# Jackie-Chou/MC-CNN-python

Measured on AMD Instinct MI355X. Metric: Mdisparities/s (HxWxD / s) end-to-end match.py timed region, images resident in HBM, higher is better.
Workload: dtype f32; 1 GPU; cfg2: 750x500 synthetic stereo pair, D=256, one pair per GPU; weights=converted reference checkpoint

## Files before the change

mc-cnn-python_amd/csrc/cost_volume.hip:

```cpp
#include "common.h"

namespace mccnn {

constexpr int CV_TW = 64;
constexpr int CV_DT = 64;
constexpr int CV_C = 64;
#ifndef CVM_WAVES_PER_SIMD
#define CVM_WAVES_PER_SIMD 6
#endif
constexpr int CV_LD = 68;

template <bool PIXEL_MAJOR>
__global__ __launch_bounds__(256) void cost_volume_exact_kernel(const float *__restrict__ fl,
                                                                const float *__restrict__ fr, int H, int W, int D,
                                                                float *__restrict__ lcv, float *__restrict__ rcv, int Dp)
{
    __shared__ __attribute__((aligned(16))) float sR[(CV_TW + CV_DT - 1) * CV_LD];
    __shared__ __attribute__((aligned(16))) float sL[CV_TW * CV_LD];
    const int w0 = blockIdx.x * CV_TW, h = blockIdx.y, d0 = blockIdx.z * CV_DT;
    if (w0 + CV_TW - 1 < d0) return;
    const int tid = threadIdx.x;
    const size_t rowbase = (size_t)h * W;
    for (int i = tid; i < CV_TW * 16; i += 256) {
        const int px = i >> 4, c4 = i & 15;
        float4 v = make_float4(0.f, 0.f, 0.f, 0.f);
        if (w0 + px < W) v = *reinterpret_cast<const float4 *>(fl + (rowbase + w0 + px) * CV_C + c4 * 4);
        *reinterpret_cast<float4 *>(&sL[px * CV_LD + c4 * 4]) = v;
    }
    const int xr0 = w0 - d0 - (CV_DT - 1);
    for (int i = tid; i < (CV_TW + CV_DT - 1) * 16; i += 256) {
        const int r = i >> 4, c4 = i & 15;
        const int x = xr0 + r;
        float4 v = make_float4(0.f, 0.f, 0.f, 0.f);
        if (x >= 0 && x < W) v = *reinterpret_cast<const float4 *>(fr + (rowbase + x) * CV_C + c4 * 4);
        *reinterpret_cast<float4 *>(&sR[r * CV_LD + c4 * 4]) = v;
    }
    __syncthreads();

    const int wl = tid & 63, dq = tid >> 6;
    const int w = w0 + wl;
    float a[CV_C];
#pragma unroll
    for (int c4 = 0; c4 < 16; ++c4) {
        const float4 v = *reinterpret_cast<const float4 *>(&sL[wl * CV_LD + c4 * 4]);
        a[c4 * 4 + 0] = v.x; a[c4 * 4 + 1] = v.y; a[c4 * 4 + 2] = v.z; a[c4 * 4 + 3] = v.w;
    }
    const size_t plane = (size_t)H * W;
    constexpr int TP = 65;
    float *const sT = sL;
    if (PIXEL_MAJOR) __syncthreads();
    for (int k = 0; k < 16; ++k) {
        const int d = d0 + dq * 16 + k;
        if (d >= D) break;
        const int r = wl + (CV_DT - 1) - (dq * 16 + k);
        if (w < W && w >= d) {
            const float *b = &sR[r * CV_LD];
            float acc[8];
#pragma unroll
            for (int i = 0; i < 8; ++i) {
                const float4 b0 = *reinterpret_cast<const float4 *>(b + i * 8);
                const float4 b1 = *reinterpret_cast<const float4 *>(b + i * 8 + 4);
                const float p0 = a[i * 8 + 0] * b0.x, p1 = a[i * 8 + 1] * b0.y, p2 = a[i * 8 + 2] * b0.z,
                            p3 = a[i * 8 + 3] * b0.w, p4 = a[i * 8 + 4] * b1.x, p5 = a[i * 8 + 5] * b1.y,
                            p6 = a[i * 8 + 6] * b1.z, p7 = a[i * 8 + 7] * b1.w;
                if (i == 0) {
                    acc[0] = p0; acc[1] = p1; acc[2] = p2; acc[3] = p3;
                    acc[4] = p4; acc[5] = p5; acc[6] = p6; acc[7] = p7;
                } else {
                    acc[0] += p0; acc[1] += p1; acc[2] += p2; acc[3] += p3;
                    acc[4] += p4; acc[5] += p5; acc[6] += p6; acc[7] += p7;
                }
            }
            float s = ((acc[0] + acc[1]) + (acc[2] + acc[3])) + ((acc[4] + acc[5]) + (acc[6] + acc[7]));
            s = 0.f + s;
            s = -1.f * s;
            if (PIXEL_MAJOR) {
                sT[wl * TP + dq * 16 + k] = s;
            } else {
                lcv[(size_t)d * plane + rowbase + w] = s;
                rcv[(size_t)d * plane + rowbase + (w - d)] = s;
            }
        }
    }
    if (PIXEL_MAJOR) {
        __syncthreads();
        const int nd = min(CV_DT, D - d0);
        const int dl = tid & 63;
        for (int px = tid >> 6; px < CV_TW; px += 4) {
            const int ww = w0 + px, d = d0 + dl;
            if (ww < W && dl < nd && ww >= d) lcv[(rowbase + ww) * (size_t)Dp + d] = sT[px * TP + dl];
        }
        for (int xi = tid >> 6; xi < CV_TW + CV_DT - 1; xi += 4) {
            const int x = xr0 + xi, d = d0 + dl, px = x + d - w0;
            if (x >= 0 && dl < nd && px >= 0 && px < CV_TW && w0 + px < W)
                rcv[(rowbase + x) * (size_t)Dp + d] = sT[px * TP + dl];
        }
    }
}

constexpr int CVP_TW = 63;
#ifndef CVP_ABL
#define CVP_ABL 0
#endif
__device__ __forceinline__ bool cvp_never(int D) { return D == 12345; }
__global__ __launch_bounds__(256, 3) void cost_volume_exact_pairs_kernel(const float *__restrict__ fl,
                                                                         const float *__restrict__ fr, int H, int W, int D,
                                                                         float *__restrict__ lcv, float *__restrict__ rcv,
                                                                         int Dp)
{
    constexpr int RING = 128;
    __shared__ __attribute__((aligned(16))) float sR[RING * CV_LD];
    __shared__ __attribute__((aligned(16))) float sL[CV_TW * CV_LD];
    const int w0 = (int)blockIdx.x * CVP_TW - 1, h = blockIdx.y;
    const int tid = threadIdx.x;
    const size_t rowbase = (size_t)h * W;
    for (int i = tid; i < CV_TW * 16; i += 256) {
        const int px = i >> 4, c4 = i & 15;
        float4 v = make_float4(0.f, 0.f, 0.f, 0.f);
        if (w0 + px >= 0 && w0 + px < W) v = *reinterpret_cast<const float4 *>(fl + (rowbase + w0 + px) * CV_C + c4 * 4);
        *reinterpret_cast<float4 *>(&sL[px * CV_LD + c4 * 4]) = v;
    }
    for (int i = tid; i < (CV_TW + CV_DT - 1) * 16; i += 256) {
        const int x = w0 - (CV_DT - 1) + (i >> 4), c4 = i & 15;
        float4 v = make_float4(0.f, 0.f, 0.f, 0.f);
        if (x >= 0 && x < W) v = *reinterpret_cast<const float4 *>(fr + (rowbase + x) * CV_C + c4 * 4);
        *reinterpret_cast<float4 *>(&sR[(x & (RING - 1)) * CV_LD + c4 * 4]) = v;
    }
    __syncthreads();

    const int wl = tid & 63, dq = tid >> 6;
    const int w = w0 + wl;
    float a[CV_C];
#pragma unroll
    for (int c4 = 0; c4 < 16; ++c4) {
        const float4 v = *reinterpret_cast<const float4 *>(&sL[wl * CV_LD + c4 * 4]);
        a[c4 * 4 + 0] = v.x; a[c4 * 4 + 1] = v.y; a[c4 * 4 + 2] = v.z; a[c4 * 4 + 3] = v.w;
    }
    constexpr int TP = CV_LD;
    float *const sT = sL;
    __syncthreads();
#pragma unroll 1
    for (int d0 = 0; d0 < D && w0 + CV_TW - 1 >= d0; d0 += CV_DT) {
        const bool more = d0 + CV_DT < D && w0 + CV_TW - 1 >= d0 + CV_DT;
        float4 nx[4];
#pragma unroll
        for (int q = 0; q < 4; ++q) {
            const int i = tid + q * 256, x = w0 - d0 - (2 * CV_DT - 1) + (i >> 4), c4 = i & 15;
            nx[q] = make_float4(0.f, 0.f, 0.f, 0.f);
            if (more && x >= 0 && x < W) nx[q] = *reinterpret_cast<const float4 *>(fr + (rowbase + x) * CV_C + c4 * 4);
        }
#pragma unroll 1
        for (int kk = 0; kk < (((CVP_ABL & 1) && !cvp_never(D)) ? 0 : 8); ++kk) {
            const int dloc = dq * 16 + 2 * kk;
            const int r = (w - d0 - dloc) & (RING - 1);
            const float *b = &sR[r * CV_LD];
            float acc[8], acn[8];
            float4 n0 = *reinterpret_cast<const float4 *>(b), n1 = *reinterpret_cast<const float4 *>(b + 4);
#pragma unroll
            for (int i = 0; i < 8; ++i) {
                const float bv[8] = {n0.x, n0.y, n0.z, n0.w, n1.x, n1.y, n1.z, n1.w};
                if (i < 7) {
                    n0 = *reinterpret_cast<const float4 *>(b + (i + 1) * 8);
                    n1 = *reinterpret_cast<const float4 *>(b + (i + 1) * 8 + 4);
                }
#pragma unroll
                for (int j = 0; j < 8; j += 4) {
                    if (i == 0) {
                        asm volatile("v_mul_f32 %0, %8, %12\n\tv_mul_f32 %1, %9, %13\n\tv_mul_f32 %2, %10, %14\n\tv_mul_f32 %3, %11, %15\n\t"
                                     "v_mul_f32_dpp %4, %12, %8 wave_shr:1 row_mask:0xf bank_mask:0xf bound_ctrl:1\n\t"
                                     "v_mul_f32_dpp %5, %13, %9 wave_shr:1 row_mask:0xf bank_mask:0xf bound_ctrl:1\n\t"
                                     "v_mul_f32_dpp %6, %14, %10 wave_shr:1 row_mask:0xf bank_mask:0xf bound_ctrl:1\n\t"
                                     "v_mul_f32_dpp %7, %15, %11 wave_shr:1 row_mask:0xf bank_mask:0xf bound_ctrl:1"
                                     : "=&v"(acc[j]), "=&v"(acc[j + 1]), "=&v"(acc[j + 2]), "=&v"(acc[j + 3]),
                                       "=&v"(acn[j]), "=&v"(acn[j + 1]), "=&v"(acn[j + 2]), "=&v"(acn[j + 3])
                                     : "v"(a[j]), "v"(a[j + 1]), "v"(a[j + 2]), "v"(a[j + 3]),
                                       "v"(bv[j]), "v"(bv[j + 1]), "v"(bv[j + 2]), "v"(bv[j + 3]));
                    } else {
                        float t0, t1, t2, t3;
                        asm volatile("v_mul_f32 %8, %12, %16\n\tv_mul_f32 %9, %13, %17\n\tv_mul_f32 %10, %14, %18\n\tv_mul_f32 %11, %15, %19\n\t"
                                     "v_add_f32 %0, %0, %8\n\tv_add_f32 %1, %1, %9\n\tv_add_f32 %2, %2, %10\n\tv_add_f32 %3, %3, %11\n\t"
                                     "v_mul_f32_dpp %8, %16, %12 wave_shr:1 row_mask:0xf bank_mask:0xf bound_ctrl:1\n\t"
                                     "v_mul_f32_dpp %9, %17, %13 wave_shr:1 row_mask:0xf bank_mask:0xf bound_ctrl:1\n\t"
                                     "v_mul_f32_dpp %10, %18, %14 wave_shr:1 row_mask:0xf bank_mask:0xf bound_ctrl:1\n\t"
                                     "v_mul_f32_dpp %11, %19, %15 wave_shr:1 row_mask:0xf bank_mask:0xf bound_ctrl:1\n\t"
                                     "v_add_f32 %4, %4, %8\n\tv_add_f32 %5, %5, %9\n\tv_add_f32 %6, %6, %10\n\tv_add_f32 %7, %7, %11"
                                     : "+v"(acc[j]), "+v"(acc[j + 1]), "+v"(acc[j + 2]), "+v"(acc[j + 3]),
                                       "+v"(acn[j]), "+v"(acn[j + 1]), "+v"(acn[j + 2]), "+v"(acn[j + 3]),
                                       "=&v"(t0), "=&v"(t1), "=&v"(t2), "=&v"(t3)
                                     : "v"(a[i * 8 + j]), "v"(a[i * 8 + j + 1]), "v"(a[i * 8 + j + 2]), "v"(a[i * 8 + j + 3]),
                                       "v"(bv[j]), "v"(bv[j + 1]), "v"(bv[j + 2]), "v"(bv[j + 3]));
                    }
                }
                __builtin_amdgcn_sched_barrier(0);
            }
            float s = ((acc[0] + acc[1]) + (acc[2] + acc[3])) + ((acc[4] + acc[5]) + (acc[6] + acc[7]));
            float sn = ((acn[0] + acn[1]) + (acn[2] + acn[3])) + ((acn[4] + acn[5]) + (acn[6] + acn[7]));
            s = 0.f + s;
            sn = 0.f + sn;
            s = -1.f * s;
            sn = -1.f * sn;
            const int d = d0 + dloc;
            if (wl >= 1 && w < W) {
                if (d < D && w >= d) sT[wl * TP + dloc] = s;
                if (d + 1 < D && w >= d + 1) sT[wl * TP + dloc + 1] = sn;
            }
        }
        __syncthreads();
#pragma unroll
        for (int q = 0; q < 4; ++q) {
            const int i = tid + q * 256, x = w0 - d0 - (2 * CV_DT - 1) + (i >> 4), c4 = i & 15;
            if (more) *reinterpret_cast<float4 *>(&sR[(x & (RING - 1)) * CV_LD + c4 * 4]) = nx[q];
        }
        const int nd = ((CVP_ABL & 2) && !cvp_never(D)) ? 0 : min(CV_DT, D - d0);
        const int xr0 = w0 - d0 - (CV_DT - 1);
        const int q4 = (tid & 15) * 4, sub = tid >> 4;
        for (int px = 1 + sub; px < CV_TW; px += 16) {
            const int ww = w0 + px, d = d0 + q4;
            if (ww >= W || q4 >= nd || ww < d) continue;
            const float4 v = *reinterpret_cast<const float4 *>(&sT[px * TP + q4]);
            float *dst = lcv + (rowbase + ww) * (size_t)Dp + d;
            if (q4 + 3 < nd && ww >= d + 3) {
                *reinterpret_cast<float4 *>(dst) = v;
            } else {
                const float e[4] = {v.x, v.y, v.z, v.w};
#pragma unroll
                for (int j = 0; j < 4; ++j)
                    if (q4 + j < nd && ww >= d + j) dst[j] = e[j];
            }
        }
        for (int xi = sub; xi < CV_TW + CV_DT - 1; xi += 16) {
            const int x = xr0 + xi, d = d0 + q4, px = x + d - w0;
            if (x < 0 || q4 >= nd || px + 3 < 1 || px >= CV_TW) continue;
            float *dst = rcv + (rowbase + x) * (size_t)Dp + d;
            if (q4 + 3 < nd && px >= 1 && px + 3 < CV_TW && w0 + px + 3 < W) {
                float4 v;
                v.x = sT[px * TP + q4];
                v.y = sT[(px + 1) * TP + q4 + 1];
                v.z = sT[(px + 2) * TP + q4 + 2];
                v.w = sT[(px + 3) * TP + q4 + 3];
                *reinterpret_cast<float4 *>(dst) = v;
            } else {
#pragma unroll
                for (int j = 0; j < 4; ++j)
                    if (q4 + j < nd && px + j >= 1 && px + j < CV_TW && w0 + px + j < W) dst[j] = sT[(px + j) * TP + q4 + j];
            }
        }
        __syncthreads();
    }
}

using f32x16 = __attribute__((ext_vector_type(16))) float;
typedef _Float16 cv_h8 __attribute__((ext_vector_type(8)));
typedef _Float16 cv_h4 __attribute__((ext_vector_type(4)));
constexpr int CVM_SP = 144;
constexpr int CVM_TP = 68;

__device__ __forceinline__ void cv_split4(const float4 v, cv_h4 &hi, cv_h4 &lo)
{
    const float x[4] = {__builtin_amdgcn_fmed3f(v.x * 1024.f, -65504.f, 65504.f),
                        __builtin_amdgcn_fmed3f(v.y * 1024.f, -65504.f, 65504.f),
                        __builtin_amdgcn_fmed3f(v.z * 1024.f, -65504.f, 65504.f),
                        __builtin_amdgcn_fmed3f(v.w * 1024.f, -65504.f, 65504.f)};
#pragma unroll
    for (int j = 0; j < 4; ++j) {
        const _Float16 h = (_Float16)x[j];
        hi[j] = h;
        lo[j] = (_Float16)(x[j] - (float)h);
    }
}

template <bool PIXEL_MAJOR>
__global__ __launch_bounds__(256, CVM_WAVES_PER_SIMD) void cost_volume_mfma_kernel(
    const float *__restrict__ fl, const float *__restrict__ fr, int H, int W, int D, float *__restrict__ lcv,
    float *__restrict__ rcv, int nwt, int nbands, int total, int Dp)
{
    constexpr int LDS_BYTES = (2 * 64 * CVM_SP > 64 * CVM_TP * 4) ? 2 * 64 * CVM_SP : 64 * CVM_TP * 4;
    __shared__ __attribute__((aligned(16))) char lds[LDS_BYTES];
    char *oL = lds, *oR = lds + 64 * CVM_SP;
    float *sT = reinterpret_cast<float *>(lds);
    int id;
    {
        const int b = blockIdx.x, qq = total >> 3, r = total & 7, xc = b & 7;
        id = (xc < r ? xc * (qq + 1) : r * (qq + 1) + (xc - r) * qq) + (b >> 3);
    }
    const int wt = id % nwt, band = (id / nwt) % nbands;
    const int h = id / (nwt * nbands);
    const int w0 = wt * 64;
    const int x0 = w0 - band * 64;
    if (x0 + 63 < 0) return;
    if (w0 - x0 - 63 >= D) return;
    const int tid = threadIdx.x;
    const size_t rowbase = (size_t)h * W;
    float4 vl[2][2], vr[2][2];
#pragma unroll
    for (int hf = 0; hf < 2; ++hf)
#pragma unroll
        for (int j = 0; j < 2; ++j) {
            const int p = j * 256 + tid, px = p >> 3, c4 = hf * 8 + (p & 7);
            vl[hf][j] = make_float4(0.f, 0.f, 0.f, 0.f);
            vr[hf][j] = make_float4(0.f, 0.f, 0.f, 0.f);
            if (w0 + px < W) vl[hf][j] = *reinterpret_cast<const float4 *>(fl + (rowbase + w0 + px) * CV_C + c4 * 4);
            const int x = x0 + px;
            if (x >= 0 && x < W) vr[hf][j] = *reinterpret_cast<const float4 *>(fr + (rowbase + x) * CV_C + c4 * 4);
        }
    const int wave = tid >> 6, lane = tid & 63;
    const int wr = (wave >> 1) * 32, wc = (wave & 1) * 32;
    f32x16 acc, acc2;
#pragma unroll
    for (int i = 0; i < 16; ++i) acc[i] = 0.f, acc2[i] = 0.f;
    const char *pa = oL + (wr + (lane & 31)) * CVM_SP + 16 * (lane >> 5);
    const char *pb = oR + (wc + (lane & 31)) * CVM_SP + 16 * (lane >> 5);
#pragma unroll
    for (int hf = 0; hf < 2; ++hf) {
        if (hf) __syncthreads();
#pragma unroll
        for (int j = 0; j < 2; ++j) {
            const int p = j * 256 + tid, px = p >> 3, c = p & 7;
            const int off = px * CVM_SP + (c >> 2) * 64 + (c & 3) * 8;
            cv_h4 hh, ll;
            cv_split4(vl[hf][j], hh, ll);
            *reinterpret_cast<cv_h4 *>(oL + off) = hh;
            *reinterpret_cast<cv_h4 *>(oL + off + 32) = ll;
            cv_split4(vr[hf][j], hh, ll);
            *reinterpret_cast<cv_h4 *>(oR + off) = hh;
            *reinterpret_cast<cv_h4 *>(oR + off + 32) = ll;
        }
        __syncthreads();
#pragma unroll
        for (int q = 0; q < 2; ++q) {
            const cv_h8 a_hi = *reinterpret_cast<const cv_h8 *>(pa + q * 64);
            const cv_h8 a_lo = *reinterpret_cast<const cv_h8 *>(pa + q * 64 + 32);
            const cv_h8 b_hi = *reinterpret_cast<const cv_h8 *>(pb + q * 64);
            const cv_h8 b_lo = *reinterpret_cast<const cv_h8 *>(pb + q * 64 + 32);
            acc2 = __builtin_amdgcn_mfma_f32_32x32x16_f16(a_lo, b_hi, acc2, 0, 0, 0);
            acc = __builtin_amdgcn_mfma_f32_32x32x16_f16(a_hi, b_hi, acc, 0, 0, 0);
            acc2 = __builtin_amdgcn_mfma_f32_32x32x16_f16(a_hi, b_lo, acc2, 0, 0, 0);
        }
    }
    __syncthreads();
    if (PIXEL_MAJOR) {
        constexpr int TP = 65;
#pragma unroll
        for (int rg = 0; rg < 16; ++rg) {
            const int row = wr + (rg & 3) + 8 * (rg >> 2) + 4 * (lane >> 5);
            const int col = wc + (lane & 31);
            sT[row * TP + col] = (acc[rg] + acc2[rg]) * (-1.f / 1048576.f);
        }
        __syncthreads();
        const int dbase = w0 - x0;
        for (int r = wave; r < 64; r += 4) {
            const int w = w0 + r, d = dbase + r - lane;
            if (w < W && d >= 0 && d < D && w >= d) lcv[(rowbase + w) * (size_t)Dp + d] = sT[r * TP + lane];
        }
        for (int c = wave; c < 64; c += 4) {
            const int x = x0 + c, d = dbase + lane - c;
            if (x >= 0 && w0 + lane < W && d >= 0 && d < D) rcv[(rowbase + x) * (size_t)Dp + d] = sT[lane * TP + c];
        }
        return;
    }
#pragma unroll
    for (int rg = 0; rg < 16; ++rg) {
        const int row = wr + (rg & 3) + 8 * (rg >> 2) + 4 * (lane >> 5);
        const int col = wc + (lane & 31);
        sT[((row - col) & 63) * CVM_TP + row] = (acc[rg] + acc2[rg]) * (-1.f / 1048576.f);
    }
    __syncthreads();
    const size_t plane = (size_t)H * W;
    const int dbase = w0 - x0;
    typedef float f4u __attribute__((ext_vector_type(4), aligned(4)));
    const int q = lane & 15, sub = lane >> 4;
    for (int rgp = wave; rgp < 16; rgp += 4) {
        const int row = rgp * 4 + sub;
        const int wl = 4 * q;
        const float4 t = *reinterpret_cast<const float4 *>(&sT[row * CVM_TP + wl]);
        const float v[4] = {t.x, t.y, t.z, t.w};
        const int w = w0 + wl;
        if (wl >= row || wl + 3 < row) {
            const int dd = wl >= row ? row : row - 64;
            const int d = dbase + dd;
            if (d < 0 || d >= D || w >= W) continue;
            float *pl = lcv + (size_t)d * plane + rowbase + w;
            float *pr = rcv + (size_t)d * plane + rowbase + (w - d);
            if (w + 3 < W) {
                f4u o;
                o[0] = v[0]; o[1] = v[1]; o[2] = v[2]; o[3] = v[3];
                *reinterpret_cast<f4u *>(pl) = o;
                *reinterpret_cast<f4u *>(pr) = o;
            } else {
#pragma unroll
                for (int j = 0; j < 4; ++j)
                    if (w + j < W) {
                        pl[j] = v[j];
                        pr[j] = v[j];
                    }
            }
        }
    }
    {
        const int row = tid >> 2, j = tid & 3;
        const int c = (row & ~3) + j;
        const int d = dbase + (c >= row ? row : row - 64);
        const int w = w0 + c;
        if ((row & 3) != 0 && d >= 0 && d < D && w < W) {
            const float v = sT[row * CVM_TP + c];
            lcv[(size_t)d * plane + rowbase + w] = v;
            rcv[(size_t)d * plane + rowbase + (w - d)] = v;
        }
    }
}

__global__ __launch_bounds__(64) void cost_volume_fill_kernel(float *__restrict__ lcv, float *__restrict__ rcv, int D,
                                                              int H, int W)
{
    __shared__ float tile[64 * 65];
    const int lane = threadIdx.x;
    const int d = D - 1 - blockIdx.y;
    const int h0 = blockIdx.x * 64;
    const int h = min(h0 + lane, H - 1);
    const int nrows = min(64, H - h0);
    if (blockIdx.z == 0) {
        float *L = lcv + ((size_t)d * H + h) * W;
        float x1 = L[d], x2 = L[d + 1], x3 = L[d + 2];
        for (int wtop = d - 1; wtop >= 0; wtop -= 64) {
            const int cnt = min(64, wtop + 1);
            for (int j = 0; j < cnt; ++j) {
                float s = 0.f - x1;
                s = s - x2;
                s = s - x3;
                const float v = -(s / 3.f);
                tile[lane * 65 + j] = v;
                x3 = x2; x2 = x1; x1 = v;
            }
            __syncthreads();
            if (lane < cnt)
                for (int r = 0; r < nrows; ++r)
                    lcv[((size_t)d * H + h0 + r) * W + (wtop - lane)] = tile[r * 65 + lane];
            __syncthreads();
        }
    } else {
        float *Rr = rcv + ((size_t)d * H + h) * W;
        float x1 = Rr[W - d - 3], x2 = Rr[W - d - 2], x3 = Rr[W - d - 1];
        for (int wbot = W - d; wbot < W; wbot += 64) {
            const int cnt = min(64, W - wbot);
            for (int j = 0; j < cnt; ++j) {
                float s = 0.f - x1;
                s = s - x2;
                s = s - x3;
                const float v = -(s / 3.f);
                tile[lane * 65 + j] = v;
                x1 = x2; x2 = x3; x3 = v;
            }
            __syncthreads();
            if (lane < cnt)
                for (int r = 0; r < nrows; ++r)
                    rcv[((size_t)d * H + h0 + r) * W + (wbot + lane)] = tile[r * 65 + lane];
            __syncthreads();
        }
    }
}

typedef uint32_t cv_u32x4 __attribute__((ext_vector_type(4)));
template <int NG>
__global__ __launch_bounds__(64) void cost_volume_fill_hwd_kernel(float *__restrict__ lcv, float *__restrict__ rcv, int D,
                                                                  int Dp, int H, int W)
{
    constexpr int PF = 8;
    constexpr int kDrop = 0x7ffffff0;
    const int lane = threadIdx.x, h = blockIdx.x;
    const bool left = blockIdx.y == 0;
    float *row = (left ? lcv : rcv) + (size_t)h * W * Dp;
    const __amdgpu_buffer_rsrc_t rs = __builtin_amdgcn_make_buffer_rsrc(row, 0, (int)((size_t)W * Dp * 4), 0x00020000);
    const unsigned pix = (unsigned)Dp * 4u;
    const int c_first = left ? D + 1 : max(W - D - 2, 0), nsteps = left ? D + 2 : W - c_first;
    auto col = [&](int t) { return left ? c_first - t : c_first + t; };
    int dbase[NG], voff[NG];
    float x1[NG][4], x2[NG][4], x3[NG][4];
#pragma unroll
    for (int g = 0; g < NG; ++g) {
        dbase[g] = g * 256 + lane * 4;
        voff[g] = dbase[g] < Dp ? dbase[g] * 4 : kDrop;
#pragma unroll
        for (int i = 0; i < 4; ++i) x1[g][i] = x2[g][i] = x3[g][i] = 0.f;
    }
    cv_u32x4 buf[PF][NG];
    auto issue = [&](int slot, int t) {
        const unsigned so = (unsigned)col(min(t, nsteps - 1)) * pix;
#pragma unroll
        for (int g = 0; g < NG; ++g) buf[slot][g] = __builtin_amdgcn_raw_buffer_load_b128(rs, voff[g], so, 0);
    };
#pragma unroll
    for (int k = 0; k < PF; ++k) issue(k, k);
    for (int t0 = 0; t0 < nsteps; t0 += PF) {
#pragma unroll
        for (int k = 0; k < PF; ++k) {
            const int t = t0 + k;
            if (t >= nsteps) continue;
            const int c = col(t);
#pragma unroll
            for (int g = 0; g < NG; ++g) {
                const cv_u32x4 u = buf[k][g];
                const float v[4] = {__uint_as_float(u.x), __uint_as_float(u.y), __uint_as_float(u.z), __uint_as_float(u.w)};
                cv_u32x4 o;
                bool any = false;
#pragma unroll
                for (int i = 0; i < 4; ++i) {
                    const int d = dbase[g] + i;
                    const bool stored = left ? c >= d : c < W - d;
                    float s = 0.f - x1[g][i];
                    s = s - x2[g][i];
                    s = s - x3[g][i];
                    const float val = stored ? v[i] : -(s / 3.f);
                    any |= !stored && d < D;
                    if (left) { x3[g][i] = x2[g][i]; x2[g][i] = x1[g][i]; x1[g][i] = val; }
                    else      { x1[g][i] = x2[g][i]; x2[g][i] = x3[g][i]; x3[g][i] = val; }
                    o[i] = __float_as_uint(val);
                }
                buffer_store_b128<0>(o, rs, any ? voff[g] : kDrop, (unsigned)c * pix);
            }
            issue(k, t + PF);
        }
    }
}


__global__ __launch_bounds__(64) void cost_volume_fill_hwd_lanes_kernel(float *__restrict__ lcv, float *__restrict__ rcv,
                                                                        int D, int Dp, int H, int W)
{
    constexpr int PF = 16;
    constexpr int kDrop = 0x7ffffff0;
    const int lane = threadIdx.x, h = blockIdx.x;
    const bool left = blockIdx.y == 0;
    const int d = (int)blockIdx.z * 64 + lane;
    const int dmax = min((int)blockIdx.z * 64 + 63, D - 1);
    if ((int)blockIdx.z * 64 >= D) return;
    float *row = (left ? lcv : rcv) + (size_t)h * W * Dp;
    const __amdgpu_buffer_rsrc_t rs = __builtin_amdgcn_make_buffer_rsrc(row, 0, (int)((size_t)W * Dp * 4), 0x00020000);
    const unsigned pix = (unsigned)Dp * 4u;
    const int c_first = left ? dmax + 2 : max(W - dmax - 3, 0), nsteps = left ? c_first + 1 : W - c_first;
    auto col = [&](int t) { return left ? c_first - t : c_first + t; };
    const int voff = d < Dp ? d * 4 : kDrop;
    const int sto = d < D ? voff : kDrop;
    float x1 = 0.f, x2 = 0.f, x3 = 0.f;
    float buf[PF];
    const int dmin = (int)blockIdx.z * 64;
    const int nA = min(nsteps, left ? c_first - dmin + 1 : (W - dmin) - c_first);
    auto issue = [&](int slot, int t) {
        const int c = col(min(t, nA - 1));
        buf[slot] = __uint_as_float(__builtin_amdgcn_raw_buffer_load_b32(rs, voff, (unsigned)c * pix, 0));
    };
    auto third = [](float s) {
        const float zh = 0.3333333432674407958984375f;
        const float q = s * zh;
        const float r = __builtin_fmaf(-3.0f, q, s);
        const float q2 = __builtin_fmaf(r, zh, q);
        return (__builtin_fabsf(s) < __builtin_inff() && s != 0.f) ? q2 : s;
    };
    auto step = [&](int c, bool stored, float have) {
        float s = 0.f - x1;
        s = s - x2;
        s = s - x3;
        const float val = stored ? have : -third(s);
        if (left) { x3 = x2; x2 = x1; x1 = val; }
        else      { x1 = x2; x2 = x3; x3 = val; }
        __builtin_amdgcn_raw_buffer_store_b32(__float_as_uint(val), rs, stored ? kDrop : sto, (unsigned)c * pix, 0);
    };
    if (nA > 0) {
#pragma unroll
        for (int k = 0; k < PF; ++k) issue(k, k);
        for (int t0 = 0; t0 < nA; t0 += PF) {
#pragma unroll
            for (int k = 0; k < PF; ++k) {
                const int t = t0 + k;
                if (t < nA) {
                    const int c = col(t);
                    step(c, left ? c >= d : c < W - d, buf[k]);
                }
                issue(k, t + PF);
            }
        }
    }
    for (int t = max(nA, 0); t < nsteps; ++t) step(col(t), false, 0.f);
}

}

extern "C" int mccnn_cost_volume(const float *fl, const float *fr, int H, int W, int C, int D, float *lcv, float *rcv,
                                 int mode, mccnn_stream_t stream)
{
    using namespace mccnn;
    MCCNN_REQUIRE(fl && fr && lcv && rcv, MCCNN_E_INVALID, "mccnn_cost_volume: null pointer");
    MCCNN_REQUIRE(H > 0 && W > 0 && D > 0, MCCNN_E_INVALID, "mccnn_cost_volume: non-positive size");
    MCCNN_REQUIRE(C == CV_C, MCCNN_E_UNSUPPORTED, "mccnn_cost_volume: C=%d, kernels are built for 64 channels", C);
    MCCNN_REQUIRE(D <= W - 2, MCCNN_E_UNSUPPORTED,
                  "mccnn_cost_volume: D=%d needs W >= D+2 (the reference's border recurrence pf:106 is degenerate "
                  "beyond that), W=%d", D, W);
    hipStream_t s = (hipStream_t)stream;
    const dim3 block(256);
    if (mode == MCCNN_CV_EXACT) {
        const dim3 grid(cdiv(W, CV_TW), H, cdiv(D, CV_DT));
        hipLaunchKernelGGL(cost_volume_exact_kernel<false>, grid, block, 0, s, fl, fr, H, W, D, lcv, rcv, 0);
    } else if (mode == MCCNN_CV_MFMA) {
        const int nwt = cdiv(W, 64), nbands = cdiv(D + 63, 64) + 1;
        const long total = (long)nwt * nbands * H;
        MCCNN_REQUIRE(total <= 0x7fffffffL, MCCNN_E_UNSUPPORTED, "mccnn_cost_volume: %ld tiles exceed the grid", total);
        hipLaunchKernelGGL(cost_volume_mfma_kernel<false>, dim3((unsigned)total), block, 0, s, fl, fr, H, W, D, lcv, rcv, nwt,
                           nbands, (int)total, 0);
    } else {
        MCCNN_REQUIRE(false, MCCNN_E_INVALID, "mccnn_cost_volume: unknown mode %d", mode);
    }
    int rc = check_launch("mccnn_cost_volume");
    if (rc) return rc;
    if (D > 1)
        hipLaunchKernelGGL(cost_volume_fill_kernel, dim3(cdiv(H, 64), D - 1, 2), dim3(64), 0, s, lcv, rcv, D, H, W);
    return check_launch("mccnn_cost_volume(fill)");
}

extern "C" int mccnn_cost_volume_hwd(const float *fl, const float *fr, int H, int W, int C, int D, float *lcv_hwd,
                                     float *rcv_hwd, int mode, mccnn_stream_t stream)
{
    using namespace mccnn;
    MCCNN_REQUIRE(fl && fr && lcv_hwd && rcv_hwd, MCCNN_E_INVALID, "mccnn_cost_volume_hwd: null pointer");
    MCCNN_REQUIRE(H > 0 && W > 0 && D > 0, MCCNN_E_INVALID, "mccnn_cost_volume_hwd: non-positive size");
    MCCNN_REQUIRE(C == CV_C, MCCNN_E_UNSUPPORTED, "mccnn_cost_volume_hwd: C=%d, kernels are built for 64 channels", C);
    MCCNN_REQUIRE(D <= W - 2, MCCNN_E_UNSUPPORTED,
                  "mccnn_cost_volume_hwd: D=%d needs W >= D+2 (the reference's border recurrence pf:106 is degenerate "
                  "beyond that), W=%d", D, W);
    MCCNN_REQUIRE(mode == MCCNN_CV_EXACT || mode == MCCNN_CV_MFMA, MCCNN_E_INVALID, "mccnn_cost_volume_hwd: unknown mode %d",
                  mode);
    MCCNN_REQUIRE(D <= 512, MCCNN_E_UNSUPPORTED, "mccnn_cost_volume_hwd: D=%d > 512", D);
    const int Dp = mccnn_hwd_pitch(D);
    MCCNN_REQUIRE((size_t)W * Dp * 4 < ((size_t)1 << 31), MCCNN_E_UNSUPPORTED,
                  "mccnn_cost_volume_hwd: a %d x %d row exceeds a buffer descriptor's reach", W, D);
    hipStream_t s = (hipStream_t)stream;
    if (mode == MCCNN_CV_MFMA) {
        const int nwt = cdiv(W, 64), nbands = cdiv(D + 63, 64) + 1;
        const long total = (long)nwt * nbands * H;
        MCCNN_REQUIRE(total <= 0x7fffffffL, MCCNN_E_UNSUPPORTED, "mccnn_cost_volume_hwd: %ld tiles exceed the grid", total);
        hipLaunchKernelGGL(cost_volume_mfma_kernel<true>, dim3((unsigned)total), dim3(256), 0, s, fl, fr, H, W, D, lcv_hwd,
                           rcv_hwd, nwt, nbands, (int)total, Dp);
    } else {
#ifdef CV_HWD_TILE_KERNEL
        const dim3 grid(cdiv(W, CV_TW), H, cdiv(D, CV_DT));
        hipLaunchKernelGGL(cost_volume_exact_kernel<true>, grid, dim3(256), 0, s, fl, fr, H, W, D, lcv_hwd, rcv_hwd, Dp);
#else
        const dim3 grid(cdiv(W, CVP_TW), H, 1);
        hipLaunchKernelGGL(cost_volume_exact_pairs_kernel, grid, dim3(256), 0, s, fl, fr, H, W, D, lcv_hwd, rcv_hwd, Dp);
#endif
    }
    int rc = check_launch("mccnn_cost_volume_hwd");
    if (rc) return rc;
    if (D > 1) {
#ifdef CV_FILL_FOUR_PER_LANE
        if (Dp <= 256)
            hipLaunchKernelGGL(cost_volume_fill_hwd_kernel<1>, dim3(H, 2), dim3(64), 0, s, lcv_hwd, rcv_hwd, D, Dp, H, W);
        else
            hipLaunchKernelGGL(cost_volume_fill_hwd_kernel<2>, dim3(H, 2), dim3(64), 0, s, lcv_hwd, rcv_hwd, D, Dp, H, W);
#else
        hipLaunchKernelGGL(cost_volume_fill_hwd_lanes_kernel, dim3(H, 2, cdiv(D, 64)), dim3(64), 0, s, lcv_hwd, rcv_hwd, D, Dp,
                           H, W);
#endif
    }
    return check_launch("mccnn_cost_volume_hwd(fill)");
}
```

Measured before the change: 11340 Mdisparities/s.

## Add double-buffered rows cost-volume kernel overlapping score stores with compute

Adds a new exact cost-volume kernel that works in 32-disparity bands with two score tiles in shared memory. It interleaves the global stores of the previous band's scores (left and right volumes) with the dot-product computation of the current band, which cuts the per-band barrier-separated store phase. The shared pair-score inner loop is factored into a helper, and the old pairs kernel stays reachable behind a compile flag. The trade-off is more loop iterations, smaller tiles, and extra bounds logic in the store path.

```diff
diff --git a/mc-cnn-python_amd/csrc/cost_volume.hip b/mc-cnn-python_amd/csrc/cost_volume.hip
--- a/mc-cnn-python_amd/csrc/cost_volume.hip
+++ b/mc-cnn-python_amd/csrc/cost_volume.hip
@@ -103,6 +103,56 @@
 #define CVP_ABL 0
 #endif
 __device__ __forceinline__ bool cvp_never(int D) { return D == 12345; }
+
+__device__ __forceinline__ void cvp_pair_scores(const float *b, const float (&a)[CV_C], float &s, float &sn)
+{
+    float acc[8], acn[8];
+    float4 n0 = *reinterpret_cast<const float4 *>(b), n1 = *reinterpret_cast<const float4 *>(b + 4);
+#pragma unroll
+    for (int i = 0; i < 8; ++i) {
+        const float bv[8] = {n0.x, n0.y, n0.z, n0.w, n1.x, n1.y, n1.z, n1.w};
+        if (i < 7) {
+            n0 = *reinterpret_cast<const float4 *>(b + (i + 1) * 8);
+            n1 = *reinterpret_cast<const float4 *>(b + (i + 1) * 8 + 4);
+        }
+#pragma unroll
+        for (int j = 0; j < 8; j += 4) {
+            if (i == 0) {
+                asm volatile("v_mul_f32 %0, %8, %12\n\tv_mul_f32 %1, %9, %13\n\tv_mul_f32 %2, %10, %14\n\tv_mul_f32 %3, %11, %15\n\t"
+                             "v_mul_f32_dpp %4, %12, %8 wave_shr:1 row_mask:0xf bank_mask:0xf bound_ctrl:1\n\t"
+                             "v_mul_f32_dpp %5, %13, %9 wave_shr:1 row_mask:0xf bank_mask:0xf bound_ctrl:1\n\t"
+                             "v_mul_f32_dpp %6, %14, %10 wave_shr:1 row_mask:0xf bank_mask:0xf bound_ctrl:1\n\t"
+                             "v_mul_f32_dpp %7, %15, %11 wave_shr:1 row_mask:0xf bank_mask:0xf bound_ctrl:1"
+                             : "=&v"(acc[j]), "=&v"(acc[j + 1]), "=&v"(acc[j + 2]), "=&v"(acc[j + 3]),
+                               "=&v"(acn[j]), "=&v"(acn[j + 1]), "=&v"(acn[j + 2]), "=&v"(acn[j + 3])
+                             : "v"(a[j]), "v"(a[j + 1]), "v"(a[j + 2]), "v"(a[j + 3]),
+                               "v"(bv[j]), "v"(bv[j + 1]), "v"(bv[j + 2]), "v"(bv[j + 3]));
+            } else {
+                float t0, t1, t2, t3;
+                asm volatile("v_mul_f32 %8, %12, %16\n\tv_mul_f32 %9, %13, %17\n\tv_mul_f32 %10, %14, %18\n\tv_mul_f32 %11, %15, %19\n\t"
+                             "v_add_f32 %0, %0, %8\n\tv_add_f32 %1, %1, %9\n\tv_add_f32 %2, %2, %10\n\tv_add_f32 %3, %3, %11\n\t"
+                             "v_mul_f32_dpp %8, %16, %12 wave_shr:1 row_mask:0xf bank_mask:0xf bound_ctrl:1\n\t"
+                             "v_mul_f32_dpp %9, %17, %13 wave_shr:1 row_mask:0xf bank_mask:0xf bound_ctrl:1\n\t"
+                             "v_mul_f32_dpp %10, %18, %14 wave_shr:1 row_mask:0xf bank_mask:0xf bound_ctrl:1\n\t"
+                             "v_mul_f32_dpp %11, %19, %15 wave_shr:1 row_mask:0xf bank_mask:0xf bound_ctrl:1\n\t"
+                             "v_add_f32 %4, %4, %8\n\tv_add_f32 %5, %5, %9\n\tv_add_f32 %6, %6, %10\n\tv_add_f32 %7, %7, %11"
+                             : "+v"(acc[j]), "+v"(acc[j + 1]), "+v"(acc[j + 2]), "+v"(acc[j + 3]),
+                               "+v"(acn[j]), "+v"(acn[j + 1]), "+v"(acn[j + 2]), "+v"(acn[j + 3]),
+                               "=&v"(t0), "=&v"(t1), "=&v"(t2), "=&v"(t3)
+                             : "v"(a[i * 8 + j]), "v"(a[i * 8 + j + 1]), "v"(a[i * 8 + j + 2]), "v"(a[i * 8 + j + 3]),
+                               "v"(bv[j]), "v"(bv[j + 1]), "v"(bv[j + 2]), "v"(bv[j + 3]));
+            }
+        }
+        __builtin_amdgcn_sched_barrier(0);
+    }
+    s = ((acc[0] + acc[1]) + (acc[2] + acc[3])) + ((acc[4] + acc[5]) + (acc[6] + acc[7]));
+    sn = ((acn[0] + acn[1]) + (acn[2] + acn[3])) + ((acn[4] + acn[5]) + (acn[6] + acn[7]));
+    s = 0.f + s;
+    sn = 0.f + sn;
+    s = -1.f * s;
+    sn = -1.f * sn;
+}
+
 __global__ __launch_bounds__(256, 3) void cost_volume_exact_pairs_kernel(const float *__restrict__ fl,
                                                                          const float *__restrict__ fr, int H, int W, int D,
                                                                          float *__restrict__ lcv, float *__restrict__ rcv,
@@ -153,52 +203,8 @@
         for (int kk = 0; kk < (((CVP_ABL & 1) && !cvp_never(D)) ? 0 : 8); ++kk) {
             const int dloc = dq * 16 + 2 * kk;
             const int r = (w - d0 - dloc) & (RING - 1);
-            const float *b = &sR[r * CV_LD];
-            float acc[8], acn[8];
-            float4 n0 = *reinterpret_cast<const float4 *>(b), n1 = *reinterpret_cast<const float4 *>(b + 4);
-#pragma unroll
-            for (int i = 0; i < 8; ++i) {
-                const float bv[8] = {n0.x, n0.y, n0.z, n0.w, n1.x, n1.y, n1.z, n1.w};
-                if (i < 7) {
-                    n0 = *reinterpret_cast<const float4 *>(b + (i + 1) * 8);
-                    n1 = *reinterpret_cast<const float4 *>(b + (i + 1) * 8 + 4);
-                }
-#pragma unroll
-                for (int j = 0; j < 8; j += 4) {
-                    if (i == 0) {
-                        asm volatile("v_mul_f32 %0, %8, %12\n\tv_mul_f32 %1, %9, %13\n\tv_mul_f32 %2, %10, %14\n\tv_mul_f32 %3, %11, %15\n\t"
-                                     "v_mul_f32_dpp %4, %12, %8 wave_shr:1 row_mask:0xf bank_mask:0xf bound_ctrl:1\n\t"
-                                     "v_mul_f32_dpp %5, %13, %9 wave_shr:1 row_mask:0xf bank_mask:0xf bound_ctrl:1\n\t"
-                                     "v_mul_f32_dpp %6, %14, %10 wave_shr:1 row_mask:0xf bank_mask:0xf bound_ctrl:1\n\t"
-                                     "v_mul_f32_dpp %7, %15, %11 wave_shr:1 row_mask:0xf bank_mask:0xf bound_ctrl:1"
-                                     : "=&v"(acc[j]), "=&v"(acc[j + 1]), "=&v"(acc[j + 2]), "=&v"(acc[j + 3]),
-                                       "=&v"(acn[j]), "=&v"(acn[j + 1]), "=&v"(acn[j + 2]), "=&v"(acn[j + 3])
-                                     : "v"(a[j]), "v"(a[j + 1]), "v"(a[j + 2]), "v"(a[j + 3]),
-                                       "v"(bv[j]), "v"(bv[j + 1]), "v"(bv[j + 2]), "v"(bv[j + 3]));
-                    } else {
-                        float t0, t1, t2, t3;
-                        asm volatile("v_mul_f32 %8, %12, %16\n\tv_mul_f32 %9, %13, %17\n\tv_mul_f32 %10, %14, %18\n\tv_mul_f32 %11, %15, %19\n\t"
-                                     "v_add_f32 %0, %0, %8\n\tv_add_f32 %1, %1, %9\n\tv_add_f32 %2, %2, %10\n\tv_add_f32 %3, %3, %11\n\t"
-                                     "v_mul_f32_dpp %8, %16, %12 wave_shr:1 row_mask:0xf bank_mask:0xf bound_ctrl:1\n\t"
-                                     "v_mul_f32_dpp %9, %17, %13 wave_shr:1 row_mask:0xf bank_mask:0xf bound_ctrl:1\n\t"
-                                     "v_mul_f32_dpp %10, %18, %14 wave_shr:1 row_mask:0xf bank_mask:0xf bound_ctrl:1\n\t"
-                                     "v_mul_f32_dpp %11, %19, %15 wave_shr:1 row_mask:0xf bank_mask:0xf bound_ctrl:1\n\t"
-                                     "v_add_f32 %4, %4, %8\n\tv_add_f32 %5, %5, %9\n\tv_add_f32 %6, %6, %10\n\tv_add_f32 %7, %7, %11"
-                                     : "+v"(acc[j]), "+v"(acc[j + 1]), "+v"(acc[j + 2]), "+v"(acc[j + 3]),
-                                       "+v"(acn[j]), "+v"(acn[j + 1]), "+v"(acn[j + 2]), "+v"(acn[j + 3]),
-                                       "=&v"(t0), "=&v"(t1), "=&v"(t2), "=&v"(t3)
-                                     : "v"(a[i * 8 + j]), "v"(a[i * 8 + j + 1]), "v"(a[i * 8 + j + 2]), "v"(a[i * 8 + j + 3]),
-                                       "v"(bv[j]), "v"(bv[j + 1]), "v"(bv[j + 2]), "v"(bv[j + 3]));
-                    }
-                }
-                __builtin_amdgcn_sched_barrier(0);
-            }
-            float s = ((acc[0] + acc[1]) + (acc[2] + acc[3])) + ((acc[4] + acc[5]) + (acc[6] + acc[7]));
-            float sn = ((acn[0] + acn[1]) + (acn[2] + acn[3])) + ((acn[4] + acn[5]) + (acn[6] + acn[7]));
-            s = 0.f + s;
-            sn = 0.f + sn;
-            s = -1.f * s;
-            sn = -1.f * sn;
+            float s, sn;
+            cvp_pair_scores(&sR[r * CV_LD], a, s, sn);
             const int d = d0 + dloc;
             if (wl >= 1 && w < W) {
                 if (d < D && w >= d) sT[wl * TP + dloc] = s;
@@ -247,6 +253,126 @@
         }
         __syncthreads();
     }
+}
+
+constexpr int CVR_DT = 32;
+constexpr int CVR_TP = 34;
+constexpr int CVR_SLOTS = 5;
+
+__device__ __forceinline__ void cvr_store_slot(int s, const float *__restrict__ sP, int tid, int w0, int pd0, int D, int W,
+                                               int Dp, size_t rowbase, float *__restrict__ lcv, float *__restrict__ rcv)
+{
+    const int nd = min(CVR_DT, D - pd0);
+    if (s < 2) {
+        const int slot = tid + s * 256, px = slot >> 3, q4 = (slot & 7) * 4;
+        const int ww = w0 + px, d = pd0 + q4;
+        if (px < 1 || ww >= W || q4 >= nd || ww < d) return;
+        const float2 lo = *reinterpret_cast<const float2 *>(&sP[px * CVR_TP + q4]);
+        const float2 hi = *reinterpret_cast<const float2 *>(&sP[px * CVR_TP + q4 + 2]);
+        float *dst = lcv + (rowbase + ww) * (size_t)Dp + d;
+        if (q4 + 3 < nd && ww >= d + 3) {
+            *reinterpret_cast<float4 *>(dst) = make_float4(lo.x, lo.y, hi.x, hi.y);
+        } else {
+            const float e[4] = {lo.x, lo.y, hi.x, hi.y};
+#pragma unroll
+            for (int j = 0; j < 4; ++j)
+                if (q4 + j < nd && ww >= d + j) dst[j] = e[j];
+        }
+    } else {
+        const int slot = tid + (s - 2) * 256, xi = slot >> 3, q4 = (slot & 7) * 4;
+        const int x = w0 - pd0 - (CVR_DT - 1) + xi, d = pd0 + q4, px = xi - (CVR_DT - 1) + q4;
+        if (xi >= CV_TW + CVR_DT - 1 || x < 0 || q4 >= nd || px + 3 < 1 || px >= CV_TW) return;
+        float *dst = rcv + (rowbase + x) * (size_t)Dp + d;
+        if (q4 + 3 < nd && px >= 1 && px + 3 < CV_TW && w0 + px + 3 < W) {
+            float4 v;
+            v.x = sP[px * CVR_TP + q4];
+            v.y = sP[(px + 1) * CVR_TP + q4 + 1];
+            v.z = sP[(px + 2) * CVR_TP + q4 + 2];
+            v.w = sP[(px + 3) * CVR_TP + q4 + 3];
+            *reinterpret_cast<float4 *>(dst) = v;
+        } else {
+#pragma unroll
+            for (int j = 0; j < 4; ++j)
+                if (q4 + j < nd && px + j >= 1 && px + j < CV_TW && w0 + px + j < W) dst[j] = sP[(px + j) * CVR_TP + q4 + j];
+        }
+    }
+}
+
+__global__ __launch_bounds__(256, 3) void cost_volume_exact_rows_kernel(const float *__restrict__ fl,
+                                                                        const float *__restrict__ fr, int H, int W, int D,
+                                                                        float *__restrict__ lcv, float *__restrict__ rcv,
+                                                                        int Dp)
+{
+    constexpr int RING = 128;
+    constexpr int TILE = CV_TW * CVR_TP;
+    static_assert(2 * TILE >= CV_TW * CV_LD, "the left features live where the score tiles go");
+    static_assert((CV_TW + 2 * CVR_DT - 1) <= RING, "a tile's columns and the next tile's new ones share the ring");
+    __shared__ __attribute__((aligned(16))) float sR[RING * CV_LD];
+    __shared__ __attribute__((aligned(16))) float sT2[2 * TILE];
+    float *const sL = sT2;
+    const int w0 = (int)blockIdx.x * CVP_TW - 1, h = blockIdx.y;
+    const int tid = threadIdx.x;
+    const size_t rowbase = (size_t)h * W;
+    for (int i = tid; i < CV_TW * 16; i += 256) {
+        const int px = i >> 4, c4 = i & 15;
+        float4 v = make_float4(0.f, 0.f, 0.f, 0.f);
+        if (w0 + px >= 0 && w0 + px < W) v = *reinterpret_cast<const float4 *>(fl + (rowbase + w0 + px) * CV_C + c4 * 4);
+        *reinterpret_cast<float4 *>(&sL[px * CV_LD + c4 * 4]) = v;
+    }
+    for (int i = tid; i < (CV_TW + CVR_DT - 1) * 16; i += 256) {
+        const int x = w0 - (CVR_DT - 1) + (i >> 4), c4 = i & 15;
+        float4 v = make_float4(0.f, 0.f, 0.f, 0.f);
+        if (x >= 0 && x < W) v = *reinterpret_cast<const float4 *>(fr + (rowbase + x) * CV_C + c4 * 4);
+        *reinterpret_cast<float4 *>(&sR[(x & (RING - 1)) * CV_LD + c4 * 4]) = v;
+    }
+    __syncthreads();
+
+    const int wl = tid & 63, dq = tid >> 6;
+    const int w = w0 + wl;
+    float a[CV_C];
+#pragma unroll
+    for (int c4 = 0; c4 < 16; ++c4) {
+        const float4 v = *reinterpret_cast<const float4 *>(&sL[wl * CV_LD + c4 * 4]);
+        a[c4 * 4 + 0] = v.x; a[c4 * 4 + 1] = v.y; a[c4 * 4 + 2] = v.z; a[c4 * 4 + 3] = v.w;
+    }
+    __syncthreads();
+    int pd0 = -1;
+    int buf = 0;
+#pragma unroll 1
+    for (int d0 = 0; d0 < D && w0 + CV_TW - 1 >= d0; d0 += CVR_DT) {
+        const bool more = d0 + CVR_DT < D && w0 + CV_TW - 1 >= d0 + CVR_DT;
+        float4 nx[2];
+#pragma unroll
+        for (int q = 0; q < 2; ++q) {
+            const int i = tid + q * 256, x = w0 - d0 - (2 * CVR_DT - 1) + (i >> 4), c4 = i & 15;
+            nx[q] = make_float4(0.f, 0.f, 0.f, 0.f);
+            if (more && x >= 0 && x < W) nx[q] = *reinterpret_cast<const float4 *>(fr + (rowbase + x) * CV_C + c4 * 4);
+        }
+        float *const sT = sT2 + buf * TILE;
+        const float *const sP = sT2 + (buf ^ 1) * TILE;
+#pragma unroll
+        for (int kk = 0; kk < 4; ++kk) {
+            if (pd0 >= 0)
+                for (int s = kk + (kk >= 2); s < kk + 1 + (kk + 1 >= 2); ++s)
+                    cvr_store_slot(s, sP, tid, w0, pd0, D, W, Dp, rowbase, lcv, rcv);
+            const int dloc = dq * 8 + 2 * kk;
+            if (d0 + dloc < D) {
+                float s, sn;
+                cvp_pair_scores(&sR[((w - d0 - dloc) & (RING - 1)) * CV_LD], a, s, sn);
+                *reinterpret_cast<float2 *>(&sT[wl * CVR_TP + dloc]) = make_float2(s, sn);
+            }
+        }
+#pragma unroll
+        for (int q = 0; q < 2; ++q) {
+            const int i = tid + q * 256, x = w0 - d0 - (2 * CVR_DT - 1) + (i >> 4), c4 = i & 15;
+            if (more) *reinterpret_cast<float4 *>(&sR[(x & (RING - 1)) * CV_LD + c4 * 4]) = nx[q];
+        }
+        __syncthreads();
+        pd0 = d0;
+        buf ^= 1;
+    }
+    if (pd0 >= 0)
+        for (int s = 0; s < CVR_SLOTS; ++s) cvr_store_slot(s, sT2 + (buf ^ 1) * TILE, tid, w0, pd0, D, W, Dp, rowbase, lcv, rcv);
 }
 
 using f32x16 = __attribute__((ext_vector_type(16))) float;
@@ -642,9 +768,12 @@
 #ifdef CV_HWD_TILE_KERNEL
         const dim3 grid(cdiv(W, CV_TW), H, cdiv(D, CV_DT));
         hipLaunchKernelGGL(cost_volume_exact_kernel<true>, grid, dim3(256), 0, s, fl, fr, H, W, D, lcv_hwd, rcv_hwd, Dp);
+#elif defined(CV_HWD_PAIRS_KERNEL)
+        const dim3 grid(cdiv(W, CVP_TW), H, 1);
+        hipLaunchKernelGGL(cost_volume_exact_pairs_kernel, grid, dim3(256), 0, s, fl, fr, H, W, D, lcv_hwd, rcv_hwd, Dp);
 #else
         const dim3 grid(cdiv(W, CVP_TW), H, 1);
-        hipLaunchKernelGGL(cost_volume_exact_pairs_kernel, grid, dim3(256), 0, s, fl, fr, H, W, D, lcv_hwd, rcv_hwd, Dp);
+        hipLaunchKernelGGL(cost_volume_exact_rows_kernel, grid, dim3(256), 0, s, fl, fr, H, W, D, lcv_hwd, rcv_hwd, Dp);
 #endif
     }
     int rc = check_launch("mccnn_cost_volume_hwd");
```

Result: no change. 11420 Mdisparities/s, median of 6 (+0.7%).
